# chenglou/ai-font-renderer

Measured on AMD Instinct MI355X. Metric: glyphs/sec training (batch fwd+bwd+step), higher is better.
Workload: dtype bf16; 1 GPU; C3: 32x32 glyph MLP 32->1024->1024->1024, char+font embedding, batch 8192/GPU (BASELINE configs[2]; per-GPU shard of configs[3]); per_gpu_batch=8192, global_batch=8192, parallelism=single, params=2137152

## Files before the change

ai-font-renderer_amd/csrc/afr_api.hip:

```cpp
#include "afr_common.h"
#include "../../include/afr.h"
static_assert(AFR_LOSS_MSE == LOSS_MSE && AFR_LOSS_BCE == LOSS_BCE, "afr.h and afr_common.h name the same loss kinds");

#include <cmath>
#include <cstdarg>
#include <cstdio>
#include <cstring>
#include <map>
#include <string>
#include <utility>
#include <vector>

static thread_local char g_err[512] = "";
static int fail(int code, const char* fmt, ...) {
    va_list ap;
    va_start(ap, fmt);
    vsnprintf(g_err, sizeof g_err, fmt, ap);
    va_end(ap);
    return code;
}
#define HIPCHK(expr)                                                                          \
    do {                                                                                      \
        hipError_t e_ = (expr);                                                               \
        if (e_ != hipSuccess) return fail(AFR_EHIP, "%s: %s", #expr, hipGetErrorString(e_)); \
// ... 2289 lines not shown
}
static SheetParams sheet_op_params(const afr_sheet_params* P) {
    SheetParams sp;
    sp.pos = P->pos; sp.emb = P->emb; sp.w_in = P->w_in; sp.b_in = P->b_in; sp.w_o = P->w_o; sp.b_o = P->b_o;
    sp.ln_g = P->ln_g; sp.ln_b = P->ln_b; sp.w1 = P->w1; sp.b1 = P->b1;
    return sp;
}
static SheetDrop sheet_op_drop(const afr_sheet_dropout* drop, float* save) {
    if (!drop) return sheet_drop(0, 0, 0, 0.f, 0.f, 0.f, 0, save);
    return sheet_drop(drop->seed, drop->step, drop->rank, drop->p_embed, drop->p_attn, drop->p_fc, 1, save);
}
extern "C" size_t afr_sheet_save_floats(int B, int L) {
    return B > 0 && L > 0 ? (size_t)B * (size_t)L * AFR_SHEET_SAVE_PER_POS : 0;
}
extern "C" int afr_op_sheet_fwd(int act_dtype, const afr_sheet_params* params, const int64_t* x, int ldx, int B, int L, int max_length, int vocab,
                                float ln_eps, const afr_sheet_dropout* drop, void* z, float* save, uint32_t* err, void* stream) {
    if (int rc = sheet_op_args("afr_op_sheet_fwd", act_dtype, params, x, ldx, B, L, max_length, vocab, drop)) return rc;
    if (!z) return fail(AFR_EINVAL, "afr_op_sheet_fwd: null argument");
    DevGuard dg(device_of(z));
    SheetDims d{L, max_length, 32, 4, 64, vocab};
    HIPCHK(afr_launch_sheet_fwd(act_dtype, d, sheet_op_params(params), sheet_op_drop(drop, save), x, ldx, B, z, ln_eps, err, (hipStream_t)stream));
    return AFR_OK;
}
extern "C" int afr_op_sheet_bwd(int act_dtype, const afr_sheet_params* params, const int64_t* x, int ldx, int B, int L, int max_length, int vocab,
                                float ln_eps, const afr_sheet_dropout* drop, const void* dz, const float* save, float* slabs,
                                const afr_sheet_slab_layout* lay, void* stream) {
    const char* what = "afr_op_sheet_bwd";
    if (int rc = sheet_op_args(what, act_dtype, params, x, ldx, B, L, max_length, vocab, drop)) return rc;
    if (!dz || !slabs || !lay) return fail(AFR_EINVAL, "%s: null argument", what);
    if (lay->total < 4 || (lay->total & 3)) return fail(AFR_EINVAL, "%s: total = %d must be a positive multiple of 4 (a block zeroes its slab 16 bytes at a time)", what, lay->total);
    if ((uintptr_t)slabs & 15) return fail(AFR_EINVAL, "%s: slabs must be 16-byte aligned", what);
    const long long off[10] = {lay->pos, lay->emb, lay->w_in, lay->b_in, lay->w_o, lay->b_o, lay->ln_g, lay->ln_b, lay->w1, lay->b1};
    const long long len[10] = {(long long)max_length * 32, (long long)vocab * 32, 96 * 32, 96, 32 * 32, 32, 32, 32, 64 * 32, 64};
    for (int i = 0; i < 10; ++i) {
        if (off[i] < 0 || off[i] + len[i] > lay->total) return fail(AFR_EINVAL, "%s: tensor %d (offset %lld, %lld floats) lies outside total = %d", what, i, off[i], len[i], lay->total);
        for (int j = 0; j < i; ++j)
            if (off[i] < off[j] + len[j] && off[j] < off[i] + len[i]) return fail(AFR_EINVAL, "%s: tensors %d and %d overlap", what, j, i);
    }
    DevGuard dg(device_of(slabs));
    SheetDims d{L, max_length, 32, 4, 64, vocab};
    SheetSlabOff so{lay->pos, lay->emb, lay->w_in, lay->b_in, lay->w_o, lay->b_o, lay->ln_g, lay->ln_b, lay->w1, lay->b1, lay->total};
    HIPCHK(afr_launch_sheet_bwd(act_dtype, d, sheet_op_params(params), sheet_op_drop(drop, const_cast<float*>(save)), x, ldx, B, dz, ln_eps, slabs, so,
                                (hipStream_t)stream));
    return AFR_OK;
}

constexpr size_t GLYPH_OP_LDS_MAX = 160 * 1024;
static int glyph_op_shape(const char* what, int act_dtype, int B, int E, int vocab, int n_fonts) {
    if (act_dtype != AFR_F32 && act_dtype != AFR_BF16) return fail(AFR_EINVAL, "%s: act_dtype must be AFR_F32 or AFR_BF16, got %d", what, act_dtype);
    if (B < 1) return fail(AFR_EINVAL, "%s: B = %d must be >= 1", what, B);
    if (vocab < 1 || n_fonts < 0) return fail(AFR_EINVAL, "%s: vocab = %d, n_fonts = %d", what, vocab, n_fonts);
    if (E < 8 || E % 8) return fail(AFR_EUNSUPPORTED, "%s: E = %d must be a positive multiple of 8", what, E);
    if ((long long)(vocab + (long long)n_fonts) * E >= (1ll << 31)) return fail(AFR_EUNSUPPORTED, "%s: a table must stay below 2^31 floats", what);
    return AFR_OK;
}
static int glyph_op_n1(const char* what, int N1) {
    if (N1 < 8 || N1 % 8) return fail(AFR_EUNSUPPORTED, "%s: N1 = %d must be a positive multiple of 8", what, N1);
    return AFR_OK;
}
static int glyph_op_fold(const char* what, int E, int vocab, int n_fonts) {
    const long long K0 = (long long)E + ((long long)vocab + n_fonts + 7) / 8 * 8;
    if (K0 > 512 || E > 128) return fail(AFR_EUNSUPPORTED, "%s: K0 = %lld, E = %d: the folded first layer takes K0 <= 512 and E <= 128", what, K0, E);
    return AFR_OK;
}
static int glyph_op_lds(const char* what, size_t lds) {
    if (lds > GLYPH_OP_LDS_MAX) return fail(AFR_EUNSUPPORTED, "%s: %zu bytes of dynamic LDS requested, above 160 KiB", what, lds);
    return AFR_OK;
}
extern "C" int afr_op_glyph_embed(int act_dtype, const float* emb, const float* femb, const int64_t* x, const int64_t* font, int B, int E, int vocab,
                                  int n_fonts, void* out, uint32_t* err, void* stream) {
    const char* what = "afr_op_glyph_embed";
    if (int rc = glyph_op_shape(what, act_dtype, B, E, vocab, n_fonts)) return rc;
    if (!emb || !x || !out || !err || (n_fonts > 0 && !femb)) return fail(AFR_EINVAL, "%s: null argument", what);
    DevGuard dg(device_of(out));
    HIPCHK(afr_launch_glyph_embed(act_dtype, emb, femb, x, font, B, E, vocab, n_fonts, out, err, (hipStream_t)stream));
    return AFR_OK;
}
extern "C" int afr_op_glyph_combo(const float* emb, const float* femb, const float* W1, const float* b1, const int64_t* x, const int64_t* font, int B,
                                  int E, int N1, int vocab, int n_fonts, void* h1c, int ld1, void* h0c, int32_t* cidx, void* w1t, uint32_t* err,
                                  void* stream) {
    const char* what = "afr_op_glyph_combo";
    if (int rc = glyph_op_shape(what, AFR_BF16, B, E, vocab, n_fonts)) return rc;
    if (int rc = glyph_op_n1(what, N1)) return rc;
    const size_t lds = (size_t)(256 * (E + 1) + 2 * 4 * E) * sizeof(float);
    if (lds > 48 * 1024) return fail(AFR_EUNSUPPORTED, "%s: E = %d needs %zu bytes of staging, above the kernel's 48 KiB (E <= 40)", what, E, lds);
    if (ld1 < N1) return fail(AFR_EINVAL, "%s: ld1 = %d is below N1 = %d", what, ld1, N1);
    if ((long long)vocab * (n_fonts > 0 ? n_fonts : 1) * (long long)ld1 >= (1ll << 31)) return fail(AFR_EUNSUPPORTED, "%s: the combination table must stay below 2^31 elements", what);
    if (!emb || !W1 || !b1 || !x || !h1c || !h0c || !cidx || !err || (n_fonts > 0 && !femb)) return fail(AFR_EINVAL, "%s: null argument", what);
    if ((uintptr_t)W1 & 15) return fail(AFR_EINVAL, "%s: W1 must be 16-byte aligned", what);
    DevGuard dg(device_of(h1c));
    HIPCHK(afr_launch_glyph_combo(emb, femb, W1, b1, x, font, B, E, N1, vocab, n_fonts, nullptr, h1c, ld1, h0c, cidx, err, (hipStream_t)stream, w1t));
    return AFR_OK;
}
extern "C" int afr_op_glyph_l1_bwd(const float* slabs, int nslabs, long long slab_stride, const float* W1, int N1, int E, int vocab, int n_fonts,
                                   float* dw1, float* dtab_part, void* stream) {
    const char* what = "afr_op_glyph_l1_bwd";
    if (int rc = glyph_op_shape(what, AFR_F32, 1, E, vocab, n_fonts)) return rc;
    if (int rc = glyph_op_n1(what, N1)) return rc;
    if (int rc = glyph_op_fold(what, E, vocab, n_fonts)) return rc;
    const int K0 = afr_glyph_k0(E, vocab, n_fonts);
    if (nslabs < 1) return fail(AFR_EINVAL, "%s: nslabs = %d must be >= 1", what, nslabs);
    if (slab_stride % 4 || (nslabs > 1 && slab_stride < (long long)N1 * K0))
        return fail(AFR_EINVAL, "%s: slab_stride = %lld must be a multiple of 4 and at least N1 * K0 = %lld", what, slab_stride, (long long)N1 * K0);
    if (!slabs || !W1 || !dw1 || !dtab_part) return fail(AFR_EINVAL, "%s: null argument", what);
    if ((uintptr_t)slabs & 15) return fail(AFR_EINVAL, "%s: slabs must be 16-byte aligned", what);
    const int G = std::max(1, std::min(1024 / (8 * K0 / 4), 8));
    if (int rc = glyph_op_lds(what, ((size_t)8 * (K0 + E) + (size_t)(G - 1) * 8 * K0) * sizeof(float))) return rc;
    DevGuard dg(device_of(dw1));
    HIPCHK(afr_launch_glyph_l1_bwd(slabs, nslabs, slab_stride, W1, N1, E, vocab, n_fonts, dw1, dtab_part, (hipStream_t)stream));
    return AFR_OK;
}
extern "C" int afr_op_glyph_l1_bwd_fused(const void* d1, const void* h0, int ldh, const int32_t* h0_rowmap, const void* W1T, const int64_t* x,
                                         const int64_t* font, int B, int N1, int vocab, int n_fonts, float* slabs, void* stream) {
    const char* what = "afr_op_glyph_l1_bwd_fused";
    if (int rc = glyph_op_shape(what, AFR_BF16, B, 32, vocab, n_fonts)) return rc;
    if (int rc = glyph_op_n1(what, N1)) return rc;
    if (!afr_glyph_l1_bwd_fused_eligible(AFR_BF16, 32, N1, vocab, n_fonts))
        return fail(AFR_EUNSUPPORTED, "%s: N1 = %d, vocab + n_fonts = %d: the fused backward takes N1 a multiple of 128 in 256 .. 1024 and at most 144 table rows (E = 32)",
                    what, N1, vocab + n_fonts);
    if (ldh < 32 || ldh % 8) return fail(AFR_EINVAL, "%s: ldh = %d must be a multiple of 8, at least 32", what, ldh);
    if ((long long)B * N1 * 2 >= (1ll << 31) || (!h0_rowmap && (long long)B * ldh * 2 >= (1ll << 31)))
        return fail(AFR_EUNSUPPORTED, "%s: d1 and h0 must stay below 2 GiB", what);
    if (!d1 || !h0 || !W1T || !x || !slabs) return fail(AFR_EINVAL, "%s: null argument", what);
    if (((uintptr_t)d1 & 15) || ((uintptr_t)h0 & 15) || ((uintptr_t)W1T & 15) || ((uintptr_t)slabs & 15))
        return fail(AFR_EINVAL, "%s: d1, h0, W1T and slabs must be 16-byte aligned", what);
    if (int rc = glyph_op_lds(what, (size_t)(N1 / afr_glyph_l1_bwd_fused_split(B, N1) / 128 + 1) * 16384 + 2 * 64 * sizeof(int))) return rc;
    DevGuard dg(device_of(slabs));
    HIPCHK(afr_launch_glyph_l1_bwd_fused(d1, N1, h0, ldh, W1T, x, font, B, N1, vocab, n_fonts, slabs, (hipStream_t)stream, h0_rowmap, nullptr));
    return AFR_OK;
}
extern "C" int afr_op_glyph_embed_bwd(int act_dtype, const void* d, const int64_t* x, const int64_t* font, int B, int E, int vocab, int n_fonts,
                                      float* slabs, void* stream) {
    const char* what = "afr_op_glyph_embed_bwd";
    if (int rc = glyph_op_shape(what, act_dtype, B, E, vocab, n_fonts)) return rc;
    if (int rc = glyph_op_lds(what, afr_glyph_embed_bwd_lds_bytes(E, vocab, n_fonts))) return rc;
    if (!d || !x || !slabs) return fail(AFR_EINVAL, "%s: null argument", what);
    DevGuard dg(device_of(slabs));
    HIPCHK(afr_launch_glyph_embed_bwd(act_dtype, d, x, font, B, E, vocab, n_fonts, slabs, (hipStream_t)stream));
    return AFR_OK;
}
```

ai-font-renderer_amd/csrc/elementwise.hip:

```cpp
#include <algorithm>
#include "afr_common.h"
#include "../../include/afr.h"

int afr_glyph_k0(int E, int vocab, int n_fonts);
static inline int grid_for(long long work_items, int block, int max_blocks = 2048) {
    long long g = (work_items + block - 1) / block;
    if (g < 1) g = 1;
    if (g > max_blocks) g = max_blocks;
    return (int)g;
}

__global__ __launch_bounds__(256) void reduce_slabs_kernel(float* __restrict__ dst, const float* __restrict__ slabs,
                                                           int nslabs, long long stride, long long n, float scale,
                                                           int accumulate) {
    const long long n4 = n >> 2;
    for (long long i = blockIdx.x * 256ll + threadIdx.x; i < n4; i += (long long)gridDim.x * 256) {
        float4 a = make_float4(0.f, 0.f, 0.f, 0.f);
        for (int s = 0; s < nslabs; ++s) {
            const float4 v = *reinterpret_cast<const float4*>(slabs + s * stride + 4 * i);
            a.x += v.x; a.y += v.y; a.z += v.z; a.w += v.w;
        }
        a.x *= scale; a.y *= scale; a.z *= scale; a.w *= scale;
        float4* d = reinterpret_cast<float4*>(dst) + i;
        if (accumulate) { float4 o = *d; a.x += o.x; a.y += o.y; a.z += o.z; a.w += o.w; }
        *d = a;
    }
    for (long long i = (n4 << 2) + blockIdx.x * 256ll + threadIdx.x; i < n; i += (long long)gridDim.x * 256) {
        float a = 0.f;
        for (int s = 0; s < nslabs; ++s) a += slabs[s * stride + i];
        a *= scale;
        if (accumulate) a += dst[i];
        dst[i] = a;
    }
}
hipError_t afr_launch_reduce(float* dst, const float* slabs, int nslabs, long long slab_stride, long long n,
                             float scale, int accumulate, hipStream_t s) {
    if (n <= 0) return hipSuccess;
    hipLaunchKernelGGL(reduce_slabs_kernel, dim3(grid_for((n + 3) / 4, 256)), dim3(256), 0, s, dst, slabs, nslabs,
                       slab_stride, n, scale, accumulate);
    return hipGetLastError();
}

__device__ __forceinline__ float4 slab_sum(const float* src, long long stride, int s0, int s1) {
    float4 a = make_float4(0.f, 0.f, 0.f, 0.f);
    int s = s0;
    for (; s + 8 <= s1; s += 8) {
        float4 v[8];
#pragma unroll
        for (int u = 0; u < 8; ++u) v[u] = *reinterpret_cast<const float4*>(src + (long long)(s + u) * stride);
#pragma unroll
        for (int u = 0; u < 8; ++u) { a.x += v[u].x; a.y += v[u].y; a.z += v[u].z; a.w += v[u].w; }
    }
#pragma unroll 4
    for (; s < s1; ++s) {
        const float4 v = *reinterpret_cast<const float4*>(src + (long long)s * stride);
        a.x += v.x; a.y += v.y; a.z += v.z; a.w += v.w;
    }
    return a;
}
template <int OPT>
__device__ __forceinline__ void reduce_finish(const RTable& t, const AdamHyper& ad, const RSeg& sg, long long i, float4 a, f32x4 pp, f32x4 mm, f32x4 vv) {
    if (t.adam) {
        const long long off = (sg.dst - t.gbase) + 4 * i;
        const bf16x4 o = opt_quad<OPT>(pp, mm, vv, (f32x4){a.x, a.y, a.z, a.w}, ad);
        *reinterpret_cast<f32x4*>(t.P + off) = pp;
        *reinterpret_cast<f32x4*>(t.M + off) = mm;
        if constexpr (OPT == OPT_ADAMW) *reinterpret_cast<f32x4*>(t.V + off) = vv;
        if (t.shadow) *reinterpret_cast<bf16x4*>(t.shadow + off) = o;
        if (sg.shT) {
            const int n = (int)((4 * i) / sg.tK), k = (int)(4 * i - (long long)n * sg.tK);
#pragma unroll
            for (int r = 0; r < 4; ++r) sg.shT[(size_t)(k + r) * sg.tN + n] = (bf16_t)pp[r];
        }
    } else {
        reinterpret_cast<float4*>(sg.dst)[i] = a;
    }
}
__device__ __forceinline__ const RTable& rtable_of(const RTable& t) { return t; }
__device__ __forceinline__ const RTable& rtable_of(const RTableG& t) { return t.t; }
__device__ __forceinline__ const AdamHyper& hyper_of(const RTable& t, int) { return t.ad; }
__device__ __forceinline__ const AdamHyper& hyper_of(const RTableG& t, int si) { return t.seg_ad[si]; }
template <int OPT = OPT_ADAMW, bool GROUPS = false>
__global__ __launch_bounds__(256) void reduce_group_kernel(std::conditional_t<GROUPS, RTableG, RTable> tt) {
    const RTable& t = rtable_of(tt);
    int si = 0;
    for (int k = 1; k < t.nseg; ++k) if ((int)blockIdx.x >= t.seg[k].blk0) si = k;
    const RSeg sg = t.seg[si];
    const AdamHyper& ad = hyper_of(tt, si);
    f32x4 pp = {0.f, 0.f, 0.f, 0.f}, mm = pp, vv = pp;
    if (sg.deep) {
        __shared__ float4 part[3][64];
        const int col = threadIdx.x & 63, grp = threadIdx.x >> 6;
        const int per = (sg.nslabs + 3) >> 2;
        for (long long i0 = (long long)(blockIdx.x - sg.blk0) * 64; i0 < sg.n4; i0 += (long long)sg.nblk * 64) {
            const long long i = i0 + col;
            const bool live = i < sg.n4;
            float4 a = make_float4(0.f, 0.f, 0.f, 0.f);
            if (live) {
                if (grp == 0 && t.adam) {
                    const long long off = (sg.dst - t.gbase) + 4 * i;
                    pp = *reinterpret_cast<f32x4*>(t.P + off); mm = *reinterpret_cast<f32x4*>(t.M + off);
                    if constexpr (OPT == OPT_ADAMW) vv = *reinterpret_cast<f32x4*>(t.V + off);
                }
                const int s0 = grp * per, s1 = min(sg.nslabs, s0 + per);
                a = slab_sum(sg.src + 4 * i, sg.stride, s0, s1);
            }
            if (grp) part[grp - 1][col] = a;
            __syncthreads();
            if (grp == 0 && live) {
#pragma unroll
                for (int g = 0; g < 3; ++g) { const float4 v = part[g][col]; a.x += v.x; a.y += v.y; a.z += v.z; a.w += v.w; }
                reduce_finish<OPT>(t, ad, sg, i, a, pp, mm, vv);
            }
            __syncthreads();
        }
        return;
    }
    for (long long i = (long long)(blockIdx.x - sg.blk0) * 256 + threadIdx.x; i < sg.n4; i += (long long)sg.nblk * 256) {
        if (t.adam) {
            const long long off = (sg.dst - t.gbase) + 4 * i;
            pp = *reinterpret_cast<f32x4*>(t.P + off); mm = *reinterpret_cast<f32x4*>(t.M + off);
            if constexpr (OPT == OPT_ADAMW) vv = *reinterpret_cast<f32x4*>(t.V + off);
        }
        const float4 a = slab_sum(sg.src + 4 * i, sg.stride, 0, sg.nslabs);
        reduce_finish<OPT>(t, ad, sg, i, a, pp, mm, vv);
    }
}
void afr_rtable_add(RTable& t, float* dst, const float* src, int nslabs, long long stride, long long n) {
    if (n <= 0) return;
    if (t.nseg >= AFR_RT_MAXSEG) { t.overflow = 1; return; }
    RSeg& sg = t.seg[t.nseg];
    sg.dst = dst; sg.src = src; sg.stride = stride; sg.n4 = n / 4; sg.nslabs = nslabs; sg.blk0 = t.nblocks;
    sg.shT = nullptr; sg.tN = sg.tK = 0;
    sg.deep = nslabs >= 32;
    const int cols = sg.deep ? 64 : 256;
    long long nb = (sg.n4 + cols - 1) / cols;
    if (nb > 1024) nb = 1024;
    sg.nblk = (int)nb;
    t.nblocks += (int)nb;
    t.nseg++;
}
hipError_t afr_launch_reduce_group(const RTable& t, hipStream_t s, const AdamHyper* seg_ad) {
    if (t.overflow || (seg_ad && !t.adam)) return hipErrorInvalidValue;
    if (t.nseg == 0) return hipSuccess;
    if (seg_ad) {
        RTableG tg;
        tg.t = t;
        for (int k = 0; k < t.nseg; ++k) tg.seg_ad[k] = seg_ad[k];
        with_opt(t.kind, [&](auto opt) { hipLaunchKernelGGL((reduce_group_kernel<opt(), true>), dim3(t.nblocks), dim3(256), 0, s, tg); });
        return hipGetLastError();
    }
    with_opt(t.adam ? t.kind : OPT_ADAMW, [&](auto opt) { hipLaunchKernelGGL(reduce_group_kernel<opt()>, dim3(t.nblocks), dim3(256), 0, s, t); });
    return hipGetLastError();
}

__device__ __forceinline__ float clip_coef(float sumsq, float gscale_abs, float max_norm, float& total_norm) {
    total_norm = gscale_abs * sqrtf(sumsq);
    return fminf(1.f, max_norm / (total_norm + 1e-6f));
}
__device__ __forceinline__ float mul_rn(float a, float b) {
#pragma clang fp contract(off)
    return a * b;
}
__device__ __forceinline__ bool finite_f(float x) { return fabsf(x) <= 3.402823466e38f; }
template <bool CLIP>
__device__ __forceinline__ bool flat_clip(float& gscale, const float* __restrict__ sumsq, float max_norm) {
    if constexpr (CLIP) {
        const float ss = *sumsq;
        if (!finite_f(ss)) return false;
        float tn;
        gscale = mul_rn(gscale, clip_coef(ss, fabsf(gscale), max_norm, tn));
    }
    return true;
}
template <int OPT> __device__ __forceinline__ float flat_decay(float lr, float wd) { return OPT == OPT_LION ? 1.f - mul_rn(lr, wd) : 1.f - lr * wd; }
// ... 606 lines not shown
}
int afr_eval_blocks(long long rows, long long cols) {
    return cols <= EVAL_WAVE_COLS ? grid_for(rows, 4, AFR_EVAL_MAX_BLOCKS) : grid_for(rows, 1, AFR_EVAL_MAX_BLOCKS);
}
hipError_t afr_launch_eval_rows(int act_dtype, int loss_kind, const void* u, const void* target, int tdtype, const int* rowmap, long long rows,
                                long long cols, float* loss_rows, uint32_t* stats, uint8_t* q, hipStream_t s) {
    if (rows <= 0 || cols <= 0) return hipSuccess;
    if ((cols & 7) || cols / 8 > 0x7fffffffll || (!target && (loss_rows || stats || rowmap)) || (!loss_rows && !stats && !q)) return hipErrorInvalidValue;
    if (!loss_rows && !stats) target = nullptr;
    const dim3 g(afr_eval_blocks(rows, cols)), b(256);
    const int cols8 = (int)(cols / 8);
    auto launch = [&](auto ta, auto tt, auto tr, auto loss, auto blk, auto ht, auto hq) {
        using T = typename decltype(ta)::type;
        using TT = typename decltype(tt)::type;
        hipLaunchKernelGGL((eval_rows_kernel<T, TT, tr(), loss(), blk(), ht(), hq()>), g, b, 0, s, (const T*)u, (const TT*)target, rowmap, rows, cols8,
                           loss_rows, stats, q);
    };
    with_act(act_dtype == AFR_BF16, [&](auto ta) { with_loss(loss_kind, [&](auto loss) { with_bool(cols > EVAL_WAVE_COLS, [&](auto blk) {
        if (!target) { launch(ta, TypeTag<uint8_t>{}, std::false_type{}, loss, blk, std::false_type{}, std::true_type{}); return; }
        with_bool(tdtype == AFR_TARGET_U8, [&](auto u8) { with_bool(rowmap != nullptr, [&](auto tr) { with_bool(q != nullptr, [&](auto hq) {
            launch(ta, TypeTag<std::conditional_t<u8(), uint8_t, float>>{}, tr, loss, blk, std::true_type{}, hq);
        }); }); });
    }); }); });
    return hipGetLastError();
}

__global__ __launch_bounds__(256) void dataset_rows_kernel(const int64_t* __restrict__ rows, int B, long long n_rows,
                                                           const int64_t* __restrict__ x, const int64_t* __restrict__ font, int L, int Lc,
                                                           int* __restrict__ ridx, int64_t* __restrict__ sx, int64_t* __restrict__ sfont,
                                                           uint32_t* err_flag) {
    const int per = sx ? Lc : 1;
    const long long total = (long long)B * per;
    for (long long i = blockIdx.x * 256ll + threadIdx.x; i < total; i += (long long)gridDim.x * 256) {
        const int b = (int)(i / per), l = (int)(i - (long long)b * per);
        long long r = rows[b];
        if (r < 0 || r >= n_rows) { if (l == 0) atomicOr(err_flag, AFR_ERR_ROW); r = min(max(r, 0ll), n_rows - 1); }
        if (l == 0) {
            ridx[b] = (int)r;
            if (sx && sfont && font) sfont[b] = font[r];
        }
        if (sx) sx[(size_t)b * Lc + l] = x[(size_t)r * L + l];
    }
}
hipError_t afr_launch_dataset_rows(const int64_t* rows, int B, long long n_rows, const int64_t* x, const int64_t* font, int L, int Lc,
                                   int* ridx, int64_t* sx, int64_t* sfont, uint32_t* err_flag, hipStream_t s) {
    if (B <= 0) return hipSuccess;
    if (n_rows <= 0 || n_rows > 0x7fffffffll || (sx && (Lc <= 0 || Lc > L))) return hipErrorInvalidValue;
    hipLaunchKernelGGL(dataset_rows_kernel, dim3(grid_for((long long)B * (sx ? Lc : 1), 256)), dim3(256), 0, s, rows, B, n_rows, x, font, L, Lc,
                       ridx, sx, sfont, err_flag);
    return hipGetLastError();
}

template <typename T>
__global__ __launch_bounds__(256) void glyph_embed_kernel(const float* __restrict__ emb, const float* __restrict__ femb,
                                                          const int64_t* __restrict__ x, const int64_t* __restrict__ font,
                                                          int B, int E, int vocab, int n_fonts, T* __restrict__ out,
                                                          uint32_t* err_flag) {
    const long long total = (long long)B * E;
    for (long long i = blockIdx.x * 256ll + threadIdx.x; i < total; i += (long long)gridDim.x * 256) {
        const int b = (int)(i / E), c = (int)(i % E);
        long long xi = x[b];
        if (xi < 0 || xi >= vocab) { if (c == 0) atomicOr(err_flag, 1u); xi = min(max(xi, 0ll), (long long)vocab - 1); }
        float v = emb[xi * E + c];
        if (n_fonts > 0) {
            long long fi = font ? font[b] : 0;
            if (fi < 0 || fi >= n_fonts) { if (c == 0) atomicOr(err_flag, 1u); fi = min(max(fi, 0ll), (long long)n_fonts - 1); }
            v += femb[fi * E + c];
        }
        out[i] = (T)v;
    }
}
hipError_t afr_launch_glyph_embed(int act_dtype, const float* emb, const float* font_emb, const int64_t* x,
                                  const int64_t* font, int B, int E, int vocab, int n_fonts, void* out,
                                  uint32_t* err_flag, hipStream_t s) {
    if (B <= 0) return hipSuccess;
    dim3 g(grid_for((long long)B * E, 256)), b(256);
    if (act_dtype == AFR_BF16)
        hipLaunchKernelGGL(glyph_embed_kernel<bf16_t>, g, b, 0, s, emb, font_emb, x, font, B, E, vocab, n_fonts, (bf16_t*)out, err_flag);
    else
        hipLaunchKernelGGL(glyph_embed_kernel<float>, g, b, 0, s, emb, font_emb, x, font, B, E, vocab, n_fonts, (float*)out, err_flag);
    return hipGetLastError();
}

constexpr int GT_ROWS = 2;
__global__ __launch_bounds__(256) void glyph_table_kernel(const float* __restrict__ emb, const float* __restrict__ femb,
                                                          const float* __restrict__ W1, int vocab, int rows, int E, int N1,
                                                          float* __restrict__ table, bf16_t* __restrict__ w1t) {
    extern __shared__ float sm[];
    float* Ws = sm;
    float* tab = sm + 256 * (E + 1);
    const int r0 = blockIdx.x * GT_ROWS, n0 = blockIdx.y * 256;
    const int nn = min(256, N1 - n0), nr = min(GT_ROWS, rows - r0);
    const int E4 = E >> 2;
    for (int i = threadIdx.x; i < nn * E4; i += 256) {
        const float4 v = *reinterpret_cast<const float4*>(W1 + (size_t)n0 * E + 4 * i);
        float* d = Ws + (i / E4) * (E + 1) + 4 * (i % E4);
        d[0] = v.x; d[1] = v.y; d[2] = v.z; d[3] = v.w;
    }
    for (int i = threadIdx.x; i < nr * E; i += 256) {
        const int r = r0 + i / E, k = i % E;
        tab[i] = r < vocab ? emb[(size_t)r * E + k] : femb[(size_t)(r - vocab) * E + k];
    }
    __syncthreads();
    if ((int)threadIdx.x >= nn) return;
    const float* w = Ws + threadIdx.x * (E + 1);
    if (w1t && blockIdx.x == 0)
        for (int k = 0; k < E; ++k) w1t[(size_t)k * N1 + n0 + threadIdx.x] = (bf16_t)w[k];
    float a[GT_ROWS];
#pragma unroll
    for (int j = 0; j < GT_ROWS; ++j) a[j] = 0.f;
    for (int k = 0; k < E; ++k) {
        const float wv = w[k];
#pragma unroll
        for (int j = 0; j < GT_ROWS; ++j) a[j] = fmaf(tab[j * E + k], wv, a[j]);
    }
    for (int j = 0; j < nr; ++j) table[(size_t)(r0 + j) * N1 + n0 + threadIdx.x] = a[j];
}
template <typename T>
__device__ __forceinline__ void store8(T* q, const float (&v)[8]) {
    if constexpr (sizeof(T) == 2) {
        bf16x8 w;
#pragma unroll
        for (int r = 0; r < 8; ++r) w[r] = (bf16_t)v[r];
        __builtin_nontemporal_store(w, reinterpret_cast<bf16x8*>(q));
    } else {
        const f32x4 lo = {v[0], v[1], v[2], v[3]}, hi = {v[4], v[5], v[6], v[7]};
        __builtin_nontemporal_store(lo, reinterpret_cast<f32x4*>(q));
        __builtin_nontemporal_store(hi, reinterpret_cast<f32x4*>(q) + 1);
    }
}
template <typename T>
__global__ __launch_bounds__(256) void glyph_l1_fwd_kernel(const float* __restrict__ table, const float* __restrict__ b1,
                                                           const float* __restrict__ emb, const float* __restrict__ femb,
                                                           const int64_t* __restrict__ x, const int64_t* __restrict__ font,
                                                           int B, int E, int N1, int vocab, int n_fonts, int K0,
                                                           T* __restrict__ h0, T* __restrict__ h1, uint32_t* err_flag) {
    const int c1 = N1 >> 3, c0 = K0 >> 3;
    const int b = blockIdx.x * blockDim.y + threadIdx.y;
    if (b >= B) return;
    long long xi = x[b];
    if (xi < 0 || xi >= vocab) { if (threadIdx.x == 0) atomicOr(err_flag, 1u); xi = min(max(xi, 0ll), (long long)vocab - 1); }
    long long fi = 0;
    if (n_fonts > 0) {
        fi = font ? font[b] : 0;
        if (fi < 0 || fi >= n_fonts) { if (threadIdx.x == 0) atomicOr(err_flag, 1u); fi = min(max(fi, 0ll), (long long)n_fonts - 1); }
    }
    const float* trow_c = table + (size_t)xi * N1;
    const float* trow_f = table + (size_t)(vocab + fi) * N1;
    for (int c = threadIdx.x; c < c1; c += blockDim.x) {
        float v[8];
        const int n = 8 * c;
        const float4 a0 = *reinterpret_cast<const float4*>(trow_c + n), a1 = *reinterpret_cast<const float4*>(trow_c + n + 4);
        const float4 g0 = *reinterpret_cast<const float4*>(b1 + n), g1 = *reinterpret_cast<const float4*>(b1 + n + 4);
        v[0] = a0.x + g0.x; v[1] = a0.y + g0.y; v[2] = a0.z + g0.z; v[3] = a0.w + g0.w;
        v[4] = a1.x + g1.x; v[5] = a1.y + g1.y; v[6] = a1.z + g1.z; v[7] = a1.w + g1.w;
        if (n_fonts > 0) {
            const float4 f0 = *reinterpret_cast<const float4*>(trow_f + n), f1 = *reinterpret_cast<const float4*>(trow_f + n + 4);
            v[0] += f0.x; v[1] += f0.y; v[2] += f0.z; v[3] += f0.w; v[4] += f1.x; v[5] += f1.y; v[6] += f1.z; v[7] += f1.w;
        }
#pragma unroll
        for (int r = 0; r < 8; ++r) v[r] = fmaxf(v[r], 0.f);
        store8(h1 + (size_t)b * N1 + n, v);
    }
    for (int c = threadIdx.x; c < c0; c += blockDim.x) {
        float v[8];
        const int k0 = 8 * c;
        if (k0 < E) {
            const float* e = emb + (size_t)xi * E + k0;
            const float4 a0 = *reinterpret_cast<const float4*>(e), a1 = *reinterpret_cast<const float4*>(e + 4);
            v[0] = a0.x; v[1] = a0.y; v[2] = a0.z; v[3] = a0.w; v[4] = a1.x; v[5] = a1.y; v[6] = a1.z; v[7] = a1.w;
            if (n_fonts > 0) {
                const float* f = femb + (size_t)fi * E + k0;
                const float4 f0 = *reinterpret_cast<const float4*>(f), f1 = *reinterpret_cast<const float4*>(f + 4);
                v[0] += f0.x; v[1] += f0.y; v[2] += f0.z; v[3] += f0.w; v[4] += f1.x; v[5] += f1.y; v[6] += f1.z; v[7] += f1.w;
            }
        } else {
            const int r0 = k0 - E, hx = (int)xi, hf = n_fonts > 0 ? vocab + (int)fi : -1;
#pragma unroll
            for (int r = 0; r < 8; ++r) v[r] = (r0 + r == hx || r0 + r == hf) ? 1.f : 0.f;
        }
        store8(h0 + (size_t)b * K0 + k0, v);
    }
}
hipError_t afr_launch_glyph_l1_fwd(int act_dtype, const float* emb, const float* font_emb, const float* W1, const float* b1,
                                   const int64_t* x, const int64_t* font, int B, int E, int N1, int vocab, int n_fonts,
                                   float* table, void* h0, void* h1, uint32_t* err_flag, hipStream_t s, void* w1t) {
    if (B <= 0) return hipSuccess;
    if ((N1 & 7) || (E & 7)) return hipErrorInvalidValue;
    const int K0 = afr_glyph_k0(E, vocab, n_fonts);
    const int rows = vocab + n_fonts;
    const size_t tlds = (size_t)(256 * (E + 1) + GT_ROWS * E) * sizeof(float);
    static size_t tlds_set[16];
    int dev = 0;
    if (tlds > 48 * 1024 && hipGetDevice(&dev) == hipSuccess && (dev < 0 || dev >= 16 || tlds_set[dev] < tlds)) {
        hipError_t e = hipFuncSetAttribute((const void*)glyph_table_kernel, hipFuncAttributeMaxDynamicSharedMemorySize, (int)tlds);
        if (e != hipSuccess) return e;
        if (dev >= 0 && dev < 16) tlds_set[dev] = tlds;
    }
    hipLaunchKernelGGL(glyph_table_kernel, dim3((rows + GT_ROWS - 1) / GT_ROWS, (N1 + 255) / 256), dim3(256), tlds, s, emb, font_emb,
                       W1, vocab, rows, E, N1, table, (bf16_t*)w1t);
    int tx = 32;
    while (tx < 128 && tx < N1 / 8) tx *= 2;
    dim3 b(tx, 256 / tx), g((B + b.y - 1) / b.y);
    if (act_dtype == AFR_BF16)
        hipLaunchKernelGGL(glyph_l1_fwd_kernel<bf16_t>, g, b, 0, s, table, b1, emb, font_emb, x, font, B, E, N1, vocab, n_fonts, K0,
                           (bf16_t*)h0, (bf16_t*)h1, err_flag);
    else
        hipLaunchKernelGGL(glyph_l1_fwd_kernel<float>, g, b, 0, s, table, b1, emb, font_emb, x, font, B, E, N1, vocab, n_fonts, K0,
                           (float*)h0, (float*)h1, err_flag);
    return hipGetLastError();
}

constexpr int CB_COMBOS = 4;
__global__ __launch_bounds__(256) void glyph_combo_kernel(const float* __restrict__ W1, const float* __restrict__ b1,
                                                          const float* __restrict__ emb, const float* __restrict__ femb,
                                                          const int64_t* __restrict__ x, const int64_t* __restrict__ font,
                                                          int B, int E, int N1, int vocab, int n_fonts, int combo_blocks,
                                                          bf16_t* __restrict__ h1c, int ld1, bf16_t* __restrict__ h0c, int* __restrict__ cidx,
                                                          bf16_t* __restrict__ w1t, uint32_t* err_flag) {
    extern __shared__ float sm[];
    const int nf = max(n_fonts, 1), ncombo = vocab * nf;
    if ((int)blockIdx.x >= combo_blocks) {
        if (blockIdx.y != 0) return;
        const int b = ((int)blockIdx.x - combo_blocks) * 256 + threadIdx.x;
        if (b >= B) return;
        long long xi = x[b], fi = (n_fonts > 0 && font) ? font[b] : 0;
        if (xi < 0 || xi >= vocab) { atomicOr(err_flag, 1u); xi = min(max(xi, 0ll), (long long)vocab - 1); }
        if (n_fonts > 0 && (fi < 0 || fi >= n_fonts)) { atomicOr(err_flag, 1u); fi = min(max(fi, 0ll), (long long)n_fonts - 1); }
        cidx[b] = (int)(xi * nf + fi);
        return;
    }
    float* Ws = sm;
    float* er = sm + 256 * (E + 1);
    float* fr = er + CB_COMBOS * E;
    const int c0 = blockIdx.x * CB_COMBOS, n0 = blockIdx.y * 256;
    const int nn = min(256, N1 - n0), nc = min(CB_COMBOS, ncombo - c0);
    const int E4 = E >> 2;
    for (int i = threadIdx.x; i < nn * E4; i += 256) {
        const float4 v = *reinterpret_cast<const float4*>(W1 + (size_t)n0 * E + 4 * i);
        float* d = Ws + (i / E4) * (E + 1) + 4 * (i % E4);
        d[0] = v.x; d[1] = v.y; d[2] = v.z; d[3] = v.w;
    }
    for (int i = threadIdx.x; i < nc * E; i += 256) {
        const int c = c0 + i / E, k = i % E, xi = c / nf, fi = c - xi * nf;
        er[i] = emb[(size_t)xi * E + k];
        fr[i] = n_fonts > 0 ? femb[(size_t)fi * E + k] : 0.f;
        if (blockIdx.y == 0) h0c[(size_t)c * E + k] = (bf16_t)(n_fonts > 0 ? er[i] + fr[i] : er[i]);
    }
    __syncthreads();
    if ((int)threadIdx.x >= nn) return;
    const float* w = Ws + threadIdx.x * (E + 1);
    if (w1t && blockIdx.x == 0)
        for (int k = 0; k < E; ++k) w1t[(size_t)k * N1 + n0 + threadIdx.x] = (bf16_t)w[k];
    float tc[CB_COMBOS], tf[CB_COMBOS];
#pragma unroll
    for (int j = 0; j < CB_COMBOS; ++j) tc[j] = tf[j] = 0.f;
    for (int k = 0; k < E; ++k) {
        const float wv = w[k];
#pragma unroll
        for (int j = 0; j < CB_COMBOS; ++j) {
            tc[j] = fmaf(er[j * E + k], wv, tc[j]);
            tf[j] = fmaf(fr[j * E + k], wv, tf[j]);
        }
    }
    const float bias = b1[n0 + threadIdx.x];
    for (int j = 0; j < nc; ++j) {
        float v = tc[j] + bias;
        if (n_fonts > 0) v += tf[j];
        h1c[(size_t)(c0 + j) * ld1 + n0 + threadIdx.x] = (bf16_t)fmaxf(v, 0.f);
    }
}
hipError_t afr_launch_glyph_combo(const float* emb, const float* font_emb, const float* W1, const float* b1, const int64_t* x,
                                  const int64_t* font, int B, int E, int N1, int vocab, int n_fonts, float* table, void* h1c,
                                  int ld1, void* h0c, int* cidx, uint32_t* err_flag, hipStream_t s, void* w1t) {
    if (B <= 0) return hipSuccess;
    if ((N1 & 7) || (E & 7) || E > 256) return hipErrorInvalidValue;
    (void)table;
    const size_t lds = (size_t)(256 * (E + 1) + 2 * CB_COMBOS * E) * sizeof(float);
    if (lds > 48 * 1024) return hipErrorInvalidValue;
    const int ncombo = vocab * (n_fonts > 0 ? n_fonts : 1);
    const int combo_blocks = (ncombo + CB_COMBOS - 1) / CB_COMBOS;
    hipLaunchKernelGGL(glyph_combo_kernel, dim3(combo_blocks + (B + 255) / 256, (N1 + 255) / 256), dim3(256), lds, s, W1, b1, emb, font_emb,
                       x, font, B, E, N1, vocab, n_fonts, combo_blocks, (bf16_t*)h1c, ld1, (bf16_t*)h0c, cidx, (bf16_t*)w1t, err_flag);
    return hipGetLastError();
}

int afr_glyph_k0(int E, int vocab, int n_fonts) { return E + (vocab + n_fonts + 7) / 8 * 8; }

constexpr int GL1_ROWS = 8, GL1_NT = 1024;
__global__ __launch_bounds__(GL1_NT) void glyph_l1_bwd_kernel(const float* __restrict__ slabs, int nslabs, long long slab_stride,
                                                              const float* __restrict__ W1, int N1, int E, int R, int K0,
                                                              float* __restrict__ dw1, float* __restrict__ dtab_part) {
    extern __shared__ float sm[];
    float* S = sm;
    float* W = sm + GL1_ROWS * K0;
    float* part = W + GL1_ROWS * E;
    const int n0 = blockIdx.x * GL1_ROWS;
    const int nr = min(GL1_ROWS, N1 - n0);
    const int cnt4 = nr * K0 / 4;
    const int full4 = GL1_ROWS * K0 / 4;
    const int G = max(1, min(GL1_NT / full4, 8));
    const int g = threadIdx.x / full4, i = threadIdx.x % full4;
    if (g < G && i < cnt4) {
        const float* src = slabs + (size_t)n0 * K0 + 4 * i;
        float4 a = make_float4(0.f, 0.f, 0.f, 0.f);
#pragma unroll 4
        for (int z = g; z < nslabs; z += G) {
            const float4 v = *reinterpret_cast<const float4*>(src + (long long)z * slab_stride);
            a.x += v.x; a.y += v.y; a.z += v.z; a.w += v.w;
        }
        float* dst = g == 0 ? S : part + (size_t)(g - 1) * GL1_ROWS * K0;
        *reinterpret_cast<float4*>(dst + 4 * i) = a;
    }
    for (int j = threadIdx.x; j < nr * E; j += GL1_NT) W[j] = W1[(size_t)n0 * E + j];
    __syncthreads();
    if ((int)threadIdx.x < cnt4) {
        float4 a = *reinterpret_cast<float4*>(S + 4 * threadIdx.x);
        for (int q = 1; q < G; ++q) {
            const float4 v = *reinterpret_cast<const float4*>(part + (size_t)(q - 1) * GL1_ROWS * K0 + 4 * threadIdx.x);
            a.x += v.x; a.y += v.y; a.z += v.z; a.w += v.w;
        }
        *reinterpret_cast<float4*>(S + 4 * threadIdx.x) = a;
    }
    __syncthreads();
    for (int j = threadIdx.x; j < nr * E; j += GL1_NT) dw1[(size_t)n0 * E + j] = S[(j / E) * K0 + (j % E)];
    float* out = dtab_part + (size_t)blockIdx.x * R * E;
    for (int j = threadIdx.x; j < R * E; j += GL1_NT) {
        const int r = j / E, k = j % E;
        float a = 0.f;
        for (int q = 0; q < nr; ++q) a = fmaf(S[q * K0 + E + r], W[q * E + k], a);
        out[j] = a;
    }
}
int afr_glyph_l1_bwd_blocks(int N1) { return (N1 + GL1_ROWS - 1) / GL1_ROWS; }
hipError_t afr_launch_glyph_l1_bwd(const float* slabs, int nslabs, long long slab_stride, const float* W1, int N1, int E,
                                   int vocab, int n_fonts, float* dw1, float* dtab_part, hipStream_t s) {
    const int K0 = afr_glyph_k0(E, vocab, n_fonts);
    if (GL1_ROWS * K0 / 4 > GL1_NT) return hipErrorInvalidValue;
    const int G = std::max(1, std::min(GL1_NT / (GL1_ROWS * K0 / 4), 8));
    const size_t lds = ((size_t)GL1_ROWS * (K0 + E) + (size_t)(G - 1) * GL1_ROWS * K0) * sizeof(float);
    hipLaunchKernelGGL(glyph_l1_bwd_kernel, dim3(afr_glyph_l1_bwd_blocks(N1)), dim3(GL1_NT), lds, s, slabs, nslabs, slab_stride, W1, N1,
                       E, vocab + n_fonts, K0, dw1, dtab_part);
    return hipGetLastError();
}

constexpr int EMB_BWD_ROWS = 32;
template <typename T>
__global__ __launch_bounds__(256) void glyph_embed_bwd_kernel(const T* __restrict__ d, const int64_t* __restrict__ x,
                                                              const int64_t* __restrict__ font, int B, int E, int vocab,
                                                              int n_fonts, float* __restrict__ slabs) {
    extern __shared__ float sm[];
    const int rows_tot = vocab + n_fonts;
    const int LDT = E + 1;
    float* acc = sm;
    float* tile = sm + (size_t)rows_tot * E;
    int* ids = reinterpret_cast<int*>(tile + (size_t)EMB_BWD_ROWS * LDT);
    int* fids = ids + EMB_BWD_ROWS;
    const int b0 = blockIdx.x * EMB_BWD_ROWS;
    const int nb = min(EMB_BWD_ROWS, B - b0);
    for (int i = threadIdx.x; i < rows_tot * E; i += 256) acc[i] = 0.f;
    for (int i = threadIdx.x; i < nb * E; i += 256) tile[(i / E) * LDT + (i % E)] = (float)d[(size_t)b0 * E + i];
    if ((int)threadIdx.x < nb) {
        long long xi = x[b0 + threadIdx.x];
        ids[threadIdx.x] = (int)min(max(xi, 0ll), (long long)vocab - 1);
        long long fi = (n_fonts > 0 && font) ? font[b0 + threadIdx.x] : 0;
// ... 45 lines not shown
```

Baseline: 45.46 million glyphs/s.

## Keep W1 rows in registers for glyph table/combo kernels; double-buffer slab reduction

The glyph table and combo kernels no longer stage a 256-row W1 tile through large dynamic LDS. Each thread now loads its own W1 row straight into float4 registers and computes the dot products from there, which removes the LDS staging, its bank traffic and the large shared-memory footprint that limited occupancy. The slab reduction helper now uses 16-wide double-buffered batches so the next batch of loads is in flight while the current one is summed, and the deep-reduction group index is made wave-uniform with readfirstlane. The trade-off is higher register pressure, plus fixed caps on E (40 for combo, 128 for table).

```diff
diff --git a/ai-font-renderer_amd/csrc/afr_api.hip b/ai-font-renderer_amd/csrc/afr_api.hip
--- a/ai-font-renderer_amd/csrc/afr_api.hip
+++ b/ai-font-renderer_amd/csrc/afr_api.hip
@@ -2395,8 +2395,10 @@
     const char* what = "afr_op_glyph_combo";
     if (int rc = glyph_op_shape(what, AFR_BF16, B, E, vocab, n_fonts)) return rc;
     if (int rc = glyph_op_n1(what, N1)) return rc;
-    const size_t lds = (size_t)(256 * (E + 1) + 2 * 4 * E) * sizeof(float);
-    if (lds > 48 * 1024) return fail(AFR_EUNSUPPORTED, "%s: E = %d needs %zu bytes of staging, above the kernel's 48 KiB (E <= 40)", what, E, lds);
+    const size_t lds = (size_t)(2 * 4 * E) * sizeof(float);
+    if (lds > 2 * 4 * 40 * sizeof(float))
+        return fail(AFR_EUNSUPPORTED, "%s: E = %d needs %zu bytes for its table rows, above the kernel's %zu (E <= 40, the former 48 KiB staging limit)", what, E, lds,
+                    2 * 4 * 40 * sizeof(float));
     if (ld1 < N1) return fail(AFR_EINVAL, "%s: ld1 = %d is below N1 = %d", what, ld1, N1);
     if ((long long)vocab * (n_fonts > 0 ? n_fonts : 1) * (long long)ld1 >= (1ll << 31)) return fail(AFR_EUNSUPPORTED, "%s: the combination table must stay below 2^31 elements", what);
     if (!emb || !W1 || !b1 || !x || !h1c || !h0c || !cidx || !err || (n_fonts > 0 && !femb)) return fail(AFR_EINVAL, "%s: null argument", what);
diff --git a/ai-font-renderer_amd/csrc/elementwise.hip b/ai-font-renderer_amd/csrc/elementwise.hip
--- a/ai-font-renderer_amd/csrc/elementwise.hip
+++ b/ai-font-renderer_amd/csrc/elementwise.hip
@@ -41,22 +41,44 @@
     return hipGetLastError();
 }
 
+constexpr int RG_BATCH = 16;
+template <bool FULL>
+__device__ __forceinline__ void slab_load(f32x4 (&v)[RG_BATCH], const float* src, long long stride, int s, int s1) {
+#pragma unroll
+    for (int u = 0; u < RG_BATCH; ++u)
+        if (FULL || s + u < s1) v[u] = *reinterpret_cast<const f32x4*>(src + (long long)(s + u) * stride);
+}
+template <bool FULL>
+__device__ __forceinline__ void slab_add(f32x4& a, const f32x4 (&v)[RG_BATCH], int s, int s1) {
+#pragma unroll
+    for (int u = 0; u < RG_BATCH; ++u)
+        if (FULL || s + u < s1) a += v[u];
+}
 __device__ __forceinline__ float4 slab_sum(const float* src, long long stride, int s0, int s1) {
-    float4 a = make_float4(0.f, 0.f, 0.f, 0.f);
+    f32x4 a = {0.f, 0.f, 0.f, 0.f};
     int s = s0;
-    for (; s + 8 <= s1; s += 8) {
-        float4 v[8];
-#pragma unroll
-        for (int u = 0; u < 8; ++u) v[u] = *reinterpret_cast<const float4*>(src + (long long)(s + u) * stride);
-#pragma unroll
-        for (int u = 0; u < 8; ++u) { a.x += v[u].x; a.y += v[u].y; a.z += v[u].z; a.w += v[u].w; }
-    }
-#pragma unroll 4
-    for (; s < s1; ++s) {
-        const float4 v = *reinterpret_cast<const float4*>(src + (long long)s * stride);
-        a.x += v.x; a.y += v.y; a.z += v.z; a.w += v.w;
-    }
-    return a;
+    if (s + RG_BATCH <= s1) {
+        f32x4 v0[RG_BATCH], v1[RG_BATCH];
+        slab_load<true>(v0, src, stride, s, s1);
+        for (;;) {
+            const bool more1 = s + 2 * RG_BATCH <= s1;
+            if (more1) slab_load<true>(v1, src, stride, s + RG_BATCH, s1);
+            slab_add<true>(a, v0, s, s1);
+            s += RG_BATCH;
+            if (!more1) break;
+            const bool more0 = s + 2 * RG_BATCH <= s1;
+            if (more0) slab_load<true>(v0, src, stride, s + RG_BATCH, s1);
+            slab_add<true>(a, v1, s, s1);
+            s += RG_BATCH;
+            if (!more0) break;
+        }
+    }
+    if (s < s1) {
+        f32x4 v[RG_BATCH];
+        slab_load<false>(v, src, stride, s, s1);
+        slab_add<false>(a, v, s, s1);
+    }
+    return make_float4(a[0], a[1], a[2], a[3]);
 }
 template <int OPT>
 __device__ __forceinline__ void reduce_finish(const RTable& t, const AdamHyper& ad, const RSeg& sg, long long i, float4 a, f32x4 pp, f32x4 mm, f32x4 vv) {
@@ -90,7 +112,7 @@
     f32x4 pp = {0.f, 0.f, 0.f, 0.f}, mm = pp, vv = pp;
     if (sg.deep) {
         __shared__ float4 part[3][64];
-        const int col = threadIdx.x & 63, grp = threadIdx.x >> 6;
+        const int col = threadIdx.x & 63, grp = __builtin_amdgcn_readfirstlane(threadIdx.x >> 6);
         const int per = (sg.nslabs + 3) >> 2;
         for (long long i0 = (long long)(blockIdx.x - sg.blk0) * 64; i0 < sg.n4; i0 += (long long)sg.nblk * 64) {
             const long long i = i0 + col;
@@ -863,39 +885,63 @@
     return hipGetLastError();
 }
 
+template <int MAXQ>
+__device__ __forceinline__ void w1_row_load(const float* __restrict__ row, int E4, bool live, float4 (&w)[MAXQ]) {
+#pragma unroll
+    for (int q = 0; q < MAXQ; ++q)
+        w[q] = (live && q < E4) ? *reinterpret_cast<const float4*>(row + 4 * q) : make_float4(0.f, 0.f, 0.f, 0.f);
+}
+template <int MAXQ, int J>
+__device__ __forceinline__ void w1_row_dots(const float4 (&w)[MAXQ], int E4, const float* tab, int E, float (&a)[J]) {
+#pragma unroll
+    for (int q = 0; q < MAXQ; ++q) {
+        if (q < E4) {
+#pragma unroll
+            for (int j = 0; j < J; ++j) {
+                const float4 t = *reinterpret_cast<const float4*>(tab + j * E + 4 * q);
+                a[j] = fmaf(t.x, w[q].x, a[j]); a[j] = fmaf(t.y, w[q].y, a[j]);
+                a[j] = fmaf(t.z, w[q].z, a[j]); a[j] = fmaf(t.w, w[q].w, a[j]);
+            }
+        }
+    }
+}
+template <int MAXQ>
+__device__ __forceinline__ void w1_row_store_t(const float4 (&w)[MAXQ], int E4, bf16_t* __restrict__ col, int N1) {
+#pragma unroll
+    for (int q = 0; q < MAXQ; ++q) {
+        if (q < E4) {
+            col[(size_t)(4 * q) * N1] = (bf16_t)w[q].x; col[(size_t)(4 * q + 1) * N1] = (bf16_t)w[q].y;
+            col[(size_t)(4 * q + 2) * N1] = (bf16_t)w[q].z; col[(size_t)(4 * q + 3) * N1] = (bf16_t)w[q].w;
+        }
+    }
+}
 constexpr int GT_ROWS = 2;
+constexpr int GT_MAXQ = 32;
 __global__ __launch_bounds__(256) void glyph_table_kernel(const float* __restrict__ emb, const float* __restrict__ femb,
                                                           const float* __restrict__ W1, int vocab, int rows, int E, int N1,
                                                           float* __restrict__ table, bf16_t* __restrict__ w1t) {
-    extern __shared__ float sm[];
-    float* Ws = sm;
-    float* tab = sm + 256 * (E + 1);
+    __shared__ float4 tab4[GT_ROWS * GT_MAXQ];
+    float* tab = reinterpret_cast<float*>(tab4);
     const int r0 = blockIdx.x * GT_ROWS, n0 = blockIdx.y * 256;
     const int nn = min(256, N1 - n0), nr = min(GT_ROWS, rows - r0);
-    const int E4 = E >> 2;
-    for (int i = threadIdx.x; i < nn * E4; i += 256) {
-        const float4 v = *reinterpret_cast<const float4*>(W1 + (size_t)n0 * E + 4 * i);
-        float* d = Ws + (i / E4) * (E + 1) + 4 * (i % E4);
-        d[0] = v.x; d[1] = v.y; d[2] = v.z; d[3] = v.w;
-    }
-    for (int i = threadIdx.x; i < nr * E; i += 256) {
+    const int E4 = E >> 2, i = threadIdx.x;
+    const bool live = i < nn, trow = i < nr * E;
+    float4 w[GT_MAXQ];
+    w1_row_load(W1 + (size_t)(n0 + i) * E, E4, live, w);
+    float tv = 0.f;
+    if (trow) {
         const int r = r0 + i / E, k = i % E;
-        tab[i] = r < vocab ? emb[(size_t)r * E + k] : femb[(size_t)(r - vocab) * E + k];
-    }
-    __syncthreads();
-    if ((int)threadIdx.x >= nn) return;
-    const float* w = Ws + threadIdx.x * (E + 1);
-    if (w1t && blockIdx.x == 0)
-        for (int k = 0; k < E; ++k) w1t[(size_t)k * N1 + n0 + threadIdx.x] = (bf16_t)w[k];
+        tv = r < vocab ? emb[(size_t)r * E + k] : femb[(size_t)(r - vocab) * E + k];
+    }
+    if (trow) tab[i] = tv;
+    __syncthreads();
+    if (!live) return;
+    if (w1t && blockIdx.x == 0) w1_row_store_t(w, E4, w1t + n0 + i, N1);
     float a[GT_ROWS];
 #pragma unroll
     for (int j = 0; j < GT_ROWS; ++j) a[j] = 0.f;
-    for (int k = 0; k < E; ++k) {
-        const float wv = w[k];
-#pragma unroll
-        for (int j = 0; j < GT_ROWS; ++j) a[j] = fmaf(tab[j * E + k], wv, a[j]);
-    }
-    for (int j = 0; j < nr; ++j) table[(size_t)(r0 + j) * N1 + n0 + threadIdx.x] = a[j];
+    w1_row_dots(w, E4, tab, E, a);
+    for (int j = 0; j < nr; ++j) table[(size_t)(r0 + j) * N1 + n0 + i] = a[j];
 }
 template <typename T>
 __device__ __forceinline__ void store8(T* q, const float (&v)[8]) {
@@ -970,15 +1016,8 @@
     if ((N1 & 7) || (E & 7)) return hipErrorInvalidValue;
     const int K0 = afr_glyph_k0(E, vocab, n_fonts);
     const int rows = vocab + n_fonts;
-    const size_t tlds = (size_t)(256 * (E + 1) + GT_ROWS * E) * sizeof(float);
-    static size_t tlds_set[16];
-    int dev = 0;
-    if (tlds > 48 * 1024 && hipGetDevice(&dev) == hipSuccess && (dev < 0 || dev >= 16 || tlds_set[dev] < tlds)) {
-        hipError_t e = hipFuncSetAttribute((const void*)glyph_table_kernel, hipFuncAttributeMaxDynamicSharedMemorySize, (int)tlds);
-        if (e != hipSuccess) return e;
-        if (dev >= 0 && dev < 16) tlds_set[dev] = tlds;
-    }
-    hipLaunchKernelGGL(glyph_table_kernel, dim3((rows + GT_ROWS - 1) / GT_ROWS, (N1 + 255) / 256), dim3(256), tlds, s, emb, font_emb,
+    if (E > 4 * GT_MAXQ) return hipErrorInvalidValue;
+    hipLaunchKernelGGL(glyph_table_kernel, dim3((rows + GT_ROWS - 1) / GT_ROWS, (N1 + 255) / 256), dim3(256), 0, s, emb, font_emb,
                        W1, vocab, rows, E, N1, table, (bf16_t*)w1t);
     int tx = 32;
     while (tx < 128 && tx < N1 / 8) tx *= 2;
@@ -993,13 +1032,15 @@
 }
 
 constexpr int CB_COMBOS = 4;
+constexpr int CB_MAXQ = 10;
+static_assert(CB_COMBOS * 4 * CB_MAXQ <= 256, "one element of the block's embedding rows per thread");
 __global__ __launch_bounds__(256) void glyph_combo_kernel(const float* __restrict__ W1, const float* __restrict__ b1,
                                                           const float* __restrict__ emb, const float* __restrict__ femb,
                                                           const int64_t* __restrict__ x, const int64_t* __restrict__ font,
                                                           int B, int E, int N1, int vocab, int n_fonts, int combo_blocks,
                                                           bf16_t* __restrict__ h1c, int ld1, bf16_t* __restrict__ h0c, int* __restrict__ cidx,
                                                           bf16_t* __restrict__ w1t, uint32_t* err_flag) {
-    extern __shared__ float sm[];
+    __shared__ float4 rows4[2 * CB_COMBOS * CB_MAXQ];
     const int nf = max(n_fonts, 1), ncombo = vocab * nf;
     if ((int)blockIdx.x >= combo_blocks) {
         if (blockIdx.y != 0) return;
@@ -1011,44 +1052,40 @@
         cidx[b] = (int)(xi * nf + fi);
         return;
     }
-    float* Ws = sm;
-    float* er = sm + 256 * (E + 1);
+    float* er = reinterpret_cast<float*>(rows4);
     float* fr = er + CB_COMBOS * E;
     const int c0 = blockIdx.x * CB_COMBOS, n0 = blockIdx.y * 256;
     const int nn = min(256, N1 - n0), nc = min(CB_COMBOS, ncombo - c0);
-    const int E4 = E >> 2;
-    for (int i = threadIdx.x; i < nn * E4; i += 256) {
-        const float4 v = *reinterpret_cast<const float4*>(W1 + (size_t)n0 * E + 4 * i);
-        float* d = Ws + (i / E4) * (E + 1) + 4 * (i % E4);
-        d[0] = v.x; d[1] = v.y; d[2] = v.z; d[3] = v.w;
-    }
-    for (int i = threadIdx.x; i < nc * E; i += 256) {
-        const int c = c0 + i / E, k = i % E, xi = c / nf, fi = c - xi * nf;
-        er[i] = emb[(size_t)xi * E + k];
-        fr[i] = n_fonts > 0 ? femb[(size_t)fi * E + k] : 0.f;
-        if (blockIdx.y == 0) h0c[(size_t)c * E + k] = (bf16_t)(n_fonts > 0 ? er[i] + fr[i] : er[i]);
-    }
-    __syncthreads();
-    if ((int)threadIdx.x >= nn) return;
-    const float* w = Ws + threadIdx.x * (E + 1);
-    if (w1t && blockIdx.x == 0)
-        for (int k = 0; k < E; ++k) w1t[(size_t)k * N1 + n0 + threadIdx.x] = (bf16_t)w[k];
+    const int E4 = E >> 2, i = threadIdx.x;
+    const bool live = i < nn, trow = i < nc * E;
+    float4 w[CB_MAXQ];
+    w1_row_load(W1 + (size_t)(n0 + i) * E, E4, live, w);
+    const float bias = live ? b1[n0 + i] : 0.f;
+    float ev = 0.f, fv = 0.f;
+    int c = 0, k = 0;
+    if (trow) {
+        c = c0 + i / E; k = i % E;
+        const int xi = c / nf, fi = c - xi * nf;
+        ev = emb[(size_t)xi * E + k];
+        if (n_fonts > 0) fv = femb[(size_t)fi * E + k];
+    }
+    if (trow) {
+        er[i] = ev;
+        fr[i] = fv;
+        if (blockIdx.y == 0) h0c[(size_t)c * E + k] = (bf16_t)(n_fonts > 0 ? ev + fv : ev);
+    }
+    __syncthreads();
+    if (!live) return;
+    if (w1t && blockIdx.x == 0) w1_row_store_t(w, E4, w1t + n0 + i, N1);
     float tc[CB_COMBOS], tf[CB_COMBOS];
 #pragma unroll
     for (int j = 0; j < CB_COMBOS; ++j) tc[j] = tf[j] = 0.f;
-    for (int k = 0; k < E; ++k) {
-        const float wv = w[k];
-#pragma unroll
-        for (int j = 0; j < CB_COMBOS; ++j) {
-            tc[j] = fmaf(er[j * E + k], wv, tc[j]);
-            tf[j] = fmaf(fr[j * E + k], wv, tf[j]);
-        }
-    }
-    const float bias = b1[n0 + threadIdx.x];
+    w1_row_dots(w, E4, er, E, tc);
+    w1_row_dots(w, E4, fr, E, tf);
     for (int j = 0; j < nc; ++j) {
         float v = tc[j] + bias;
         if (n_fonts > 0) v += tf[j];
-        h1c[(size_t)(c0 + j) * ld1 + n0 + threadIdx.x] = (bf16_t)fmaxf(v, 0.f);
+        h1c[(size_t)(c0 + j) * ld1 + n0 + i] = (bf16_t)fmaxf(v, 0.f);
     }
 }
 hipError_t afr_launch_glyph_combo(const float* emb, const float* font_emb, const float* W1, const float* b1, const int64_t* x,
@@ -1057,11 +1094,10 @@
     if (B <= 0) return hipSuccess;
     if ((N1 & 7) || (E & 7) || E > 256) return hipErrorInvalidValue;
     (void)table;
-    const size_t lds = (size_t)(256 * (E + 1) + 2 * CB_COMBOS * E) * sizeof(float);
-    if (lds > 48 * 1024) return hipErrorInvalidValue;
+    if (E > 4 * CB_MAXQ) return hipErrorInvalidValue;
     const int ncombo = vocab * (n_fonts > 0 ? n_fonts : 1);
     const int combo_blocks = (ncombo + CB_COMBOS - 1) / CB_COMBOS;
-    hipLaunchKernelGGL(glyph_combo_kernel, dim3(combo_blocks + (B + 255) / 256, (N1 + 255) / 256), dim3(256), lds, s, W1, b1, emb, font_emb,
+    hipLaunchKernelGGL(glyph_combo_kernel, dim3(combo_blocks + (B + 255) / 256, (N1 + 255) / 256), dim3(256), 0, s, W1, b1, emb, font_emb,
                        x, font, B, E, N1, vocab, n_fonts, combo_blocks, (bf16_t*)h1c, ld1, (bf16_t*)h0c, cidx, (bf16_t*)w1t, err_flag);
     return hipGetLastError();
 }
```

Measured after the change: 45.85 million glyphs/s (median of 6 runs). No clear change (+0.9%).
